# lez-s/Materialist

Hardware: AMD Instinct MI355X
Metric: opt_iterations_per_sec_512x512 (higher is better)
Workload: dtype f32; 1 GPU; BASELINE configs[1] synthetic: 1x512x512/GPU, --model_name pos_mlp --opt_order 'rm a' part rm, spp 64; mode=pos_mlp, height=512, width=512, spp=64, images_per_gpu=1, light=SH25, parallelism=dp1 (independent images, no data-path collective)

## Files before the change

### materialist_amd/csrc/posmlp_kernels.hip

```cpp
#include <hip/hip_runtime.h>
#include <stdint.h>
#include <atomic>
#include <type_traits>

#include "../../include/matpbr.h"
#include "../../include/matpbr_experimental.h"
#include "posmlp_device.hpp"

namespace {


constexpr int kBM = 128, kBN = 128, kBK = 32;
constexpr int kPersistent = 512;
constexpr int EPI_SINCOS = 0, EPI_MULC = 1, EPI_BIAS = 2;

struct HeadArgs {
  const float* w;
  int ldw;
  const float* bias;
  ArmHead h;
};

__global__ __launch_bounds__(256) void mlp_tail_copy_kernel(float* __restrict__ out, int ldo, const float* __restrict__ tail, int ldt, long M, int N) {
  const int w = 256 - N;
// ... 1455 lines not shown
#pragma unroll
      for (int q = 0; q < 4; ++q) *reinterpret_cast<float4*>(sx + lane * 16 + 4 * ((q + lane) & 3)) = *reinterpret_cast<const float4*>(xs + 4 * ((q + lane) & 3));
    }
    float4 cvb[2][4];
    auto cv_load = [&](int b, float4 (&dst)[4]) {
      const float* src = p.cmul + (size_t)(row0 + wm * 64 + (b >> 2) * 32 + t_row) * p.ldo + wn * 128 + (b & 3) * 32 + t_col;
#pragma unroll
      for (int ps = 0; ps < 4; ++ps) dst[ps] = *reinterpret_cast<const float4*>(src + (size_t)(8 * ps) * p.ldo);
    };
    if (EPI == EPI_MULC) cv_load(0, cvb[0]);
    float hacc[4][5];
#pragma unroll
    for (int b = 0; b < 8; ++b) {
      const int mi = b >> 2, ni = b & 3;
      const size_t o0 = (size_t)(row0 + wm * 64 + mi * 32 + t_row) * p.ldo + wn * 128 + ni * 32 + t_col;
      if (EPI == EPI_MULC && b + 1 < 8) cv_load(b + 1, cvb[(b + 1) & 1]);
      if (HEAD && ni == 0) {
#pragma unroll
        for (int ps = 0; ps < 4; ++ps)
#pragma unroll
          for (int j = 0; j < 5; ++j) hacc[ps][j] = 0.f;
      }
      float second[16];
#pragma unroll
      for (int r = 0; r < 16; ++r) {
        float v = acc[mi][ni][r];
        if (BLK) v *= a_unscale;
        if (EPI == EPI_SINCOS) {
          const float pre = F16 ? __builtin_fmaf(v, kF16WUnscale, bn[ni]) : v + bn[ni];
          if (PK) v = sin_packed(pre);
          else sincos_cw(pre, v, second[r]);
        }
        scr[((r & 3) + 8 * (r >> 2) + 4 * lh) * kLd + li] = v;
      }
      float4 vrow[4];
#pragma unroll
      for (int ps = 0; ps < 4; ++ps) {
        float4 v = *reinterpret_cast<const float4*>(scr + (t_row + 8 * ps) * kLd + t_col);
        if (EPI == EPI_MULC) {
          float4 c4 = cvb[b & 1][ps];
          if (p.cmul_sin) c4 = cos_from_packed_sin(c4);
          v.x *= c4.x; v.y *= c4.y; v.z *= c4.z; v.w *= c4.w;
          csum4[ni].x += v.x; csum4[ni].y += v.y; csum4[ni].z += v.z; csum4[ni].w += v.w;
          if (BLK && !W0) omax = __builtin_fmaxf(__builtin_fmaxf(omax, __builtin_fmaxf(__builtin_fabsf(v.x), __builtin_fabsf(v.y))),
                                                   __builtin_fmaxf(__builtin_fabsf(v.z), __builtin_fabsf(v.w)));
        }
        if (EPI == EPI_SINCOS && !HEAD && ni == 3 && p.tail != nullptr && wn == 1) {
            const int col = 224 + t_col;
            const float* tl = p.tail + (size_t)(row0 + wm * 64 + mi * 32 + t_row + 8 * ps) * p.ldt - p.N;
            if (col >= p.N) v.x = tl[col];
            if (col + 1 >= p.N) v.y = tl[col + 1];
            if (col + 2 >= p.N) v.z = tl[col + 2];
            if (col + 3 >= p.N) v.w = tl[col + 3];
        }
        if (W0) *reinterpret_cast<float4*>(scr + (t_row + 8 * ps) * kLd + t_col) = v;
        else *reinterpret_cast<float4*>(p.out0 + o0 + (size_t)(8 * ps) * p.ldo) = v;
        vrow[ps] = v;
      }
      if (W0) {
#pragma unroll
        for (int ct = 0; ct < 2; ++ct)
#pragma unroll
          for (int kk = 0; kk < 8; ++kk)
            acc0[ni][ct] = __builtin_amdgcn_mfma_f32_16x16x4f32(scr[(4 * kk + (lane >> 4)) * kLd + 16 * ct + (lane & 15)],
                                                                sx[(mi * 32 + 4 * kk + (lane >> 4)) * 16 + (lane & 15)], acc0[ni][ct], 0, 0, 0);
      }
      if (HEAD) {
#pragma unroll
        for (int j = 0; j < 5; ++j) {
          const float4 w4 = *reinterpret_cast<const float4*>(sW4 + j * 256 + wn * 128 + ni * 32 + t_col);
#pragma unroll
          for (int ps = 0; ps < 4; ++ps)
            hacc[ps][j] = __builtin_fmaf(vrow[ps].x, w4.x, __builtin_fmaf(vrow[ps].y, w4.y, __builtin_fmaf(vrow[ps].z, w4.z, __builtin_fmaf(vrow[ps].w, w4.w, hacc[ps][j]))));
        }
      }
      if (EPI == EPI_SINCOS && !PK) {
#pragma unroll
        for (int r = 0; r < 16; ++r) scr[((r & 3) + 8 * (r >> 2) + 4 * lh) * kLd + li] = second[r];
#pragma unroll
        for (int ps = 0; ps < 4; ++ps)
          *reinterpret_cast<float4*>(p.out1 + o0 + (size_t)(8 * ps) * p.ldo) = *reinterpret_cast<const float4*>(scr + (t_row + 8 * ps) * kLd + t_col);
      }
      if (HEAD && ni == 3) {
#pragma unroll
        for (int ps = 0; ps < 4; ++ps)
#pragma unroll
          for (int j = 0; j < 5; ++j) {
            float v = hacc[ps][j];
            v = dpp_add_f<0x111>(v);
            v = dpp_add_f<0x112>(v);
            v = dpp_add_f<0x114>(v);
            if ((lane & 7) == 7) sComb[((wm * 64 + mi * 32 + t_row + 8 * ps) * 2 + wn) * 8 + j] = v;
          }
      }
    }
    if (HEAD) {
      __syncthreads();
      if (tid < kBM) {
        float v5[5];
#pragma unroll
        for (int j = 0; j < 5; ++j) v5[j] = (sComb[(tid * 2) * 8 + j] + sComb[(tid * 2 + 1) * 8 + j]) + hd.bias[j];
        arm_head_store(hd.h, (long)row0 + tid, v5);
      }
      __syncthreads();
    }
    if (BLK && !W0 && p.o_tmax != nullptr) {
      const float wmx = wave_max_lane63(omax);
      if (lane == 63) atomicMax(p.o_tmax + tile, __float_as_uint(wmx));
    }
    asm volatile("s_waitcnt lgkmcnt(0)" ::: "memory");
  }
  asm volatile("s_waitcnt vmcnt(0)" ::: "memory");
  if (W0) {
    const size_t slab = (size_t)blockIdx.x * 2 + wm;
#pragma unroll
    for (int ni = 0; ni < 4; ++ni)
#pragma unroll
      for (int ct = 0; ct < 2; ++ct)
#pragma unroll
        for (int r = 0; r < 4; ++r)
          p.w0_part[(slab * 16 + (lane & 15)) * 256 + wn * 128 + ni * 32 + 16 * ct + 4 * (lane >> 4) + r] = acc0[ni][ct][r];
  }
  if (EPI == EPI_MULC && p.colsum != nullptr) {
    float* sRed = reinterpret_cast<float*>(gx_smem);
    const int t_row = lane >> 3, t_col = (lane & 7) * 4;
    __syncthreads();
#pragma unroll
    for (int ni = 0; ni < 4; ++ni)
      *reinterpret_cast<float4*>(sRed + (wm * 8 + t_row) * 256 + wn * 128 + ni * 32 + t_col) = csum4[ni];
    __syncthreads();
    float t = 0.f;
#pragma unroll
    for (int sl = 0; sl < 16; ++sl) t += sRed[sl * 256 + tid];
    p.colsum[(size_t)blockIdx.x * 256 + tid] = t;
  }
}

constexpr int kWgStage = 2 * 3 * 2 * 256;
constexpr size_t kWgSmem = 2 * kWgStage * sizeof(uint4);
#ifndef MATPBR_WG_DEPTH
#define MATPBR_WG_DEPTH 2
#endif
constexpr int kWgDepth = MATPBR_WG_DEPTH;
constexpr int kWgThreads = 512;
__device__ __forceinline__ int wg_perm(int i) { return (i & 16) + 2 * (i & 7) + ((i >> 3) & 1); }
template <int NPROD, bool EARLY>
__device__ __forceinline__ void wgrad_bx_body(const float* __restrict__ G, int ldg, const float* __restrict__ X, int ldx,
                                              float* __restrict__ partial, long M, long rows_per_slab, uint4* sW, const unsigned* __restrict__ g_tmax) {
  constexpr bool F16 = NPROD == 3;
  constexpr int NP = F16 ? 2 : 3;
  const int tid = threadIdx.x, lane = tid & 63, wave = tid >> 6;
  const int nq = wave >> 1, kq = wave & 1, li = lane & 31, lh = lane >> 5;
  const long m_begin = (long)blockIdx.x * rows_per_slab;
  const long m_end = (m_begin + rows_per_slab < M) ? m_begin + rows_per_slab : M;
  const int steps = m_begin < m_end ? (int)((m_end - m_begin) / 16) : 0;
  float g_scale = 1.0f, g_unscale = 1.0f;
  if (F16 && steps > 0) {
    unsigned mb = 0;
    for (long t = m_begin / kBM; t <= (m_end - 1) / kBM; ++t) mb = g_tmax[t] > mb ? g_tmax[t] : mb;
    block_scale(mb, g_scale, g_unscale);
  }

  f32x16 acc[2][4];
#pragma unroll
  for (int ni = 0; ni < 2; ++ni)
#pragma unroll
    for (int ki = 0; ki < 4; ++ki)
#pragma unroll
      for (int r = 0; r < 16; ++r) acc[ni][ki][r] = 0.f;

  const int cp = tid & 255, sh = tid >> 8;
  const float* src = (cp >> 7) ? X + (m_begin + 8 * sh) * ldx + 2 * (cp & 127) : G + (m_begin + 8 * sh) * ldg + 2 * (cp & 127);
  const long ld = (cp >> 7) ? ldx : ldg;
  const float my_scale = (F16 && !(cp >> 7)) ? g_scale : 1.0f;
  uint4* sdst = sW + (((cp >> 7) * NP) * 2 + sh) * 256 + ((cp & 127) >> 3) * 16 + (cp & 7);
  float2 raw[kWgDepth][8];
  auto load_stage = [&](int slot, int step) {
#pragma unroll
    for (int j = 0; j < 8; ++j) raw[slot][j] = *reinterpret_cast<const float2*>(src + (16L * step + j) * ld);
  };
  auto split_store = [&](int slot, int buf) {
#pragma unroll
    for (int c = 0; c < 2; ++c) {
      uint4 pc[3];
      const float2* r = raw[slot];
#define MATPBR_COMP(v) (c == 0 ? (v).x : (v).y)
      if (F16) {
        split2h(MATPBR_COMP(r[0]) * my_scale, MATPBR_COMP(r[1]) * my_scale, pc[0].x, pc[1].x);
        split2h(MATPBR_COMP(r[2]) * my_scale, MATPBR_COMP(r[3]) * my_scale, pc[0].y, pc[1].y);
        split2h(MATPBR_COMP(r[4]) * my_scale, MATPBR_COMP(r[5]) * my_scale, pc[0].z, pc[1].z);
        split2h(MATPBR_COMP(r[6]) * my_scale, MATPBR_COMP(r[7]) * my_scale, pc[0].w, pc[1].w);
      } else {
        split3(MATPBR_COMP(r[0]), MATPBR_COMP(r[1]), pc[0].x, pc[1].x, pc[2].x);
        split3(MATPBR_COMP(r[2]), MATPBR_COMP(r[3]), pc[0].y, pc[1].y, pc[2].y);
        split3(MATPBR_COMP(r[4]), MATPBR_COMP(r[5]), pc[0].z, pc[1].z, pc[2].z);
        split3(MATPBR_COMP(r[6]), MATPBR_COMP(r[7]), pc[0].w, pc[1].w, pc[2].w);
      }
#undef MATPBR_COMP
#pragma unroll
      for (int piece = 0; piece < NP; ++piece) sdst[buf * kWgStage + (piece * 2) * 256 + 8 * c] = pc[piece];
    }
  };
  auto stage = [&](int slot, int buf, int next_stage) {
    __builtin_amdgcn_sched_barrier(0);
    split_store(slot, buf);
    __builtin_amdgcn_sched_barrier(0);
    load_stage(slot, next_stage < steps ? next_stage : steps - 1);
    __builtin_amdgcn_sched_barrier(0);
  };

  if (steps > 0) {
    load_stage(0, 0);
    split_store(0, 0);
#pragma unroll
    for (int d = 0; d < kWgDepth; ++d) {
      __builtin_amdgcn_sched_barrier(0);
      load_stage((1 + d) % kWgDepth, 1 + d < steps ? 1 + d : steps - 1);
    }
    __builtin_amdgcn_sched_barrier(0);
    __syncthreads();
    auto step = [&](auto u_tag, int st) {
        constexpr int u = decltype(u_tag)::value;
        const int cur = st & 1;
        if (EARLY) stage((u + 1) % kWgDepth, cur ^ 1, st + 1 + kWgDepth);
        const uint4* sa = sW + cur * kWgStage + lh * 256 + nq * 64 + li;
        const uint4* sb = sW + cur * kWgStage + (NP * 2 + lh) * 256 + kq * 128 + li;
        uint4 a[3][2];
#pragma unroll
        for (int piece = 0; piece < NP; ++piece)
#pragma unroll
          for (int ni = 0; ni < 2; ++ni) a[piece][ni] = sa[(piece * 2) * 256 + ni * 32];
#pragma unroll
        for (int kh = 0; kh < 2; ++kh) {
          uint4 b[3][2];
#pragma unroll
          for (int piece = 0; piece < NP; ++piece)
#pragma unroll
            for (int k2 = 0; k2 < 2; ++k2) b[piece][k2] = sb[(piece * 2) * 256 + (kh * 2 + k2) * 32];
          if constexpr (F16) {
#pragma unroll
            for (int t = 0; t < 3; ++t) {
              constexpr int ia[3] = {1, 0, 0}, ib[3] = {0, 1, 0};
#pragma unroll
              for (int k2 = 0; k2 < 2; ++k2)
#pragma unroll
                for (int ni = 0; ni < 2; ++ni)
                  acc[ni][kh * 2 + k2] = __builtin_amdgcn_mfma_f32_32x32x16_f16(__builtin_bit_cast(f16x8, a[ia[t]][ni]),
                                                                               __builtin_bit_cast(f16x8, b[ib[t]][k2]), acc[ni][kh * 2 + k2], 0, 0, 0);
            }
          }
#pragma unroll
          for (int t = 0; t < (F16 ? 0 : 9); ++t) {
            constexpr int ia[9] = {2, 1, 2, 2, 0, 1, 1, 0, 0}, ib[9] = {2, 2, 1, 0, 2, 1, 0, 1, 0};
            if (NPROD == 6 && t < 3) continue;
#pragma unroll
            for (int k2 = 0; k2 < 2; ++k2)
#pragma unroll
              for (int ni = 0; ni < 2; ++ni)
                acc[ni][kh * 2 + k2] = __builtin_amdgcn_mfma_f32_32x32x16_bf16(__builtin_bit_cast(bf16x8, a[ia[t]][ni]),
                                                                              __builtin_bit_cast(bf16x8, b[ib[t]][k2]), acc[ni][kh * 2 + k2], 0, 0, 0);
          }
        }
        if (!EARLY) stage((u + 1) % kWgDepth, cur ^ 1, st + 1 + kWgDepth);
        __syncthreads();
    };
    int st0 = 0;
    for (; st0 + kWgDepth <= steps; st0 += kWgDepth) {
      step(std::integral_constant<int, 0>{}, st0);
      if constexpr (kWgDepth > 1) step(std::integral_constant<int, 1>{}, st0 + 1);
      if constexpr (kWgDepth > 2) step(std::integral_constant<int, 2>{}, st0 + 2);
      if constexpr (kWgDepth > 3) step(std::integral_constant<int, 3>{}, st0 + 3);
    }
    if (st0 < steps) step(std::integral_constant<int, 0>{}, st0);
    if constexpr (kWgDepth > 2) if (st0 + 1 < steps) step(std::integral_constant<int, 1>{}, st0 + 1);
    if constexpr (kWgDepth > 3) if (st0 + 2 < steps) step(std::integral_constant<int, 2>{}, st0 + 2);
  }
  float* out = partial + (long)blockIdx.x * 256 * 256;
#pragma unroll
  for (int ni = 0; ni < 2; ++ni)
#pragma unroll
    for (int ki = 0; ki < 4; ++ki)
#pragma unroll
      for (int r = 0; r < 16; ++r) {
        const int n = nq * 64 + ni * 32 + wg_perm((r & 3) + 8 * (r >> 2) + 4 * lh);
        const int k = kq * 128 + ki * 32 + wg_perm(li);
        out[n * 256 + k] = F16 ? acc[ni][ki][r] * g_unscale : acc[ni][ki][r];
      }
}

template <int NPROD>
__global__ __launch_bounds__(kWgThreads, 1) void mlp_wgrad_bx(const float* __restrict__ G, int ldg, const float* __restrict__ X, int ldx,
                                                              float* __restrict__ partial, long M, long rows_per_slab, const unsigned* __restrict__ g_tmax) {
  extern __shared__ __align__(16) unsigned char wg_smem[];
  uint4* sW = reinterpret_cast<uint4*>(wg_smem);
  if (threadIdx.x >> 8)
    wgrad_bx_body<NPROD, true>(G, ldg, X, ldx, partial, M, rows_per_slab, sW, g_tmax);
  else
    wgrad_bx_body<NPROD, false>(G, ldg, X, ldx, partial, M, rows_per_slab, sW, g_tmax);
}

#ifndef MATPBR_WG_HX
#define MATPBR_WG_HX 1
#endif
constexpr int kHxRaw = 16 * 2 * 1024;
constexpr int kHxPieces = 2 * 2 * 2 * 256;
constexpr size_t kHxSmem = 3 * kHxRaw + kHxPieces * sizeof(uint4);
__global__ __launch_bounds__(kWgThreads, 1) void mlp_wgrad_hx(const float* __restrict__ G, int ldg, const float* __restrict__ X, int ldx,
                                                              float* __restrict__ partial, long M, long rows_per_slab, const unsigned* __restrict__ g_tmax) {
  extern __shared__ __align__(16) unsigned char hx_smem[];
  uint4* sP = reinterpret_cast<uint4*>(hx_smem + 3 * kHxRaw);
  const int tid = threadIdx.x, lane = tid & 63, wave = tid >> 6;
  const int nq = wave >> 1, kq = wave & 1, li = lane & 31, lh = lane >> 5;
  (void)rows_per_slab;
  const int tiles = (int)(M / kBM);
  const int t_first = tiles - 1 - (int)blockIdx.x;
  const int my_tiles = t_first >= 0 ? t_first / (int)gridDim.x + 1 : 0;
  const int steps = my_tiles * (kBM / 16);
  float g_scale = 1.0f, g_unscale = 1.0f;
  if (steps > 0) {
    unsigned mb = 0;
    for (int t = t_first; t >= 0; t -= (int)gridDim.x) mb = g_tmax[t] > mb ? g_tmax[t] : mb;
    block_scale(mb, g_scale, g_unscale);
  }
  f32x16 acc[2][4];
#pragma unroll
  for (int ni = 0; ni < 2; ++ni)
#pragma unroll
    for (int ki = 0; ki < 4; ++ki)
#pragma unroll
      for (int r = 0; r < 16; ++r) acc[ni][ki][r] = 0.f;
  if (steps > 0) {
    const int wave_u = __builtin_amdgcn_readfirstlane(wave);
    const bool loader = wave_u < 4;
    const unsigned lds0 = lds_byte_address(hx_smem);
    unsigned vg[4], vx[4];
#pragma unroll
    for (int j = 0; j < 4; ++j) {
      vg[j] = (unsigned)(j * ldg) * 4u + (unsigned)lane * 16u - 1024u * j;
      vx[j] = (unsigned)(j * ldx) * 4u + (unsigned)lane * 16u - 1024u * j;
    }
    auto issue = [&](int step, int buf) {
      const int sc = step < steps ? step : steps - 1;
      const long row = ((long)t_first - (long)(sc >> 3) * gridDim.x) * kBM + 16 * (7 - (sc & 7)) + 4 * wave_u;
      const unsigned dst = lds0 + (unsigned)buf * (unsigned)kHxRaw + (unsigned)wave_u * 4096u;
      glds16_x4v(G + row * ldg, vg[0], vg[1], vg[2], vg[3], dst);
      glds16_x4v(X + row * ldx, vx[0], vx[1], vx[2], vx[3], dst + 16u * 1024u);
    };
    const int cp = tid & 255, sh = tid >> 8;
    const float my_scale = (cp >> 7) ? 1.0f : g_scale;
    const unsigned raw_off = (unsigned)((cp >> 7) * 16 * 1024 + (8 * sh) * 1024 + (cp & 127) * 8);
    uint4* sdst = sP + (((cp >> 7) * 2) * 2 + sh) * 256 + ((cp & 127) >> 3) * 16 + (cp & 7);
    float2 raw[8];
    auto read_raw = [&](int buf) {
#pragma unroll
      for (int j = 0; j < 8; ++j) raw[j] = *reinterpret_cast<const float2*>(hx_smem + buf * kHxRaw + raw_off + j * 1024);
    };
    auto cut_store = [&]() {
#pragma unroll
      for (int c = 0; c < 2; ++c) {
        uint4 pc[2];
#define MATPBR_COMP(v) (c == 0 ? (v).x : (v).y)
        split2h(MATPBR_COMP(raw[0]) * my_scale, MATPBR_COMP(raw[1]) * my_scale, pc[0].x, pc[1].x);
        split2h(MATPBR_COMP(raw[2]) * my_scale, MATPBR_COMP(raw[3]) * my_scale, pc[0].y, pc[1].y);
        split2h(MATPBR_COMP(raw[4]) * my_scale, MATPBR_COMP(raw[5]) * my_scale, pc[0].z, pc[1].z);
        split2h(MATPBR_COMP(raw[6]) * my_scale, MATPBR_COMP(raw[7]) * my_scale, pc[0].w, pc[1].w);
#undef MATPBR_COMP
#pragma unroll
        for (int piece = 0; piece < 2; ++piece) sdst[(piece * 2) * 256 + 8 * c] = pc[piece];
      }
    };
    auto products = [&](const uint4 (&a)[2][2], const uint4 (&b)[2][4]) {
#pragma unroll
      for (int ki = 0; ki < 4; ++ki)
#pragma unroll
        for (int t = 0; t < 3; ++t) {
          constexpr int ia[3] = {1, 0, 0}, ib[3] = {0, 1, 0};
#pragma unroll
          for (int ni = 0; ni < 2; ++ni)
            acc[ni][ki] = __builtin_amdgcn_mfma_f32_32x32x16_f16(__builtin_bit_cast(f16x8, a[ia[t]][ni]), __builtin_bit_cast(f16x8, b[ib[t]][ki]), acc[ni][ki], 0, 0, 0);
        }
    };
    if (loader) { issue(0, 0); issue(1, 1); }
    if (loader) asm volatile("s_waitcnt vmcnt(8)" ::: "memory");
    asm volatile("s_barrier" ::: "memory");
    read_raw(0);
    cut_store();
    if (loader) issue(2, 2);
    const uint4* sa = sP + lh * 256 + nq * 64 + li;
    const uint4* sb = sP + (2 * 2 + lh) * 256 + kq * 128 + li;
    int nxt = 1;
    for (int st = 0; st < steps; ++st) {
      if (loader) asm volatile("s_waitcnt vmcnt(8)" ::: "memory");
      asm volatile("s_waitcnt lgkmcnt(0)\n\ts_barrier" ::: "memory");
      uint4 a[2][2], b[2][4];
#pragma unroll
      for (int piece = 0; piece < 2; ++piece) {
#pragma unroll
        for (int ni = 0; ni < 2; ++ni) a[piece][ni] = sa[(piece * 2) * 256 + ni * 32];
#pragma unroll
        for (int ki = 0; ki < 4; ++ki) b[piece][ki] = sb[(piece * 2) * 256 + ki * 32];
      }
      read_raw(nxt);
      asm volatile("s_waitcnt lgkmcnt(0)\n\ts_barrier" ::: "memory");
      if (loader) {
        issue(st + 3, nxt == 0 ? 2 : nxt - 1);
        __builtin_amdgcn_sched_barrier(0);
      }
      products(a, b);
      cut_store();
      nxt = nxt == 2 ? 0 : nxt + 1;
    }
    asm volatile("s_waitcnt vmcnt(0)" ::: "memory");
  }
  float* out = partial + (long)blockIdx.x * 256 * 256;
#pragma unroll
  for (int ni = 0; ni < 2; ++ni)
#pragma unroll
    for (int ki = 0; ki < 4; ++ki)
#pragma unroll
      for (int r = 0; r < 16; ++r) {
        const int n = nq * 64 + ni * 32 + wg_perm((r & 3) + 8 * (r >> 2) + 4 * lh);
        const int k = kq * 128 + ki * 32 + wg_perm(li);
        out[n * 256 + k] = acc[ni][ki][r] * g_unscale;
      }
}

constexpr size_t kBxSmem = 2 * kBxStage * sizeof(uint4) + 8 * 32 * kLd * sizeof(float);
constexpr size_t kBxSmemHead = kBxSmem + (5 * 256 + 128 * 2 * 8) * sizeof(float);
std::atomic<int> g_nt_gl{2};
std::atomic<int> g_nt_w0_gx{0};
inline bool gl_ok(const NtArgs& p) {
  return g_nt_gl.load(std::memory_order_relaxed) != 0 && p.K > 32 && (long)kBM * p.lda * 4 < (1l << 31);
}
template <auto Kernel>
bool lds_opt_in(size_t bytes) {
  static std::atomic<unsigned long long> done{0};
  int dev = 0;
  if (hipGetDevice(&dev) != hipSuccess) return false;
  const unsigned long long bit = 1ull << (dev & 63);
  if (done.load(std::memory_order_acquire) & bit) return true;
  if (hipFuncSetAttribute(reinterpret_cast<const void*>(Kernel), hipFuncAttributeMaxDynamicSharedMemorySize, (int)bytes) != hipSuccess) return false;
  done.fetch_or(bit, std::memory_order_release);
  return true;
}
template <int EPI, int NPROD, bool FULL>
bool launch_nt_bx_full(const NtArgs& p, const uint4* wsplit, unsigned grid, hipStream_t stream) {
  if constexpr (FULL) if (gl_ok(p)) {
    if (!lds_opt_in<&mlp_nt_bx<EPI, NPROD, true, false, false, true>>(kGlSmem)) return false;
    hipLaunchKernelGGL((mlp_nt_bx<EPI, NPROD, true, false, false, true>), dim3(grid), dim3(kBxThreads), kGlSmem, stream, p, wsplit, HeadArgs{});
    return true;
  }
  if (!lds_opt_in<&mlp_nt_bx<EPI, NPROD, FULL>>(kBxSmem)) return false;
  hipLaunchKernelGGL((mlp_nt_bx<EPI, NPROD, FULL>), dim3(grid), dim3(kBxThreads), kBxSmem, stream, p, wsplit, HeadArgs{});
  return true;
}
constexpr size_t kBxSmemW0 = kBxSmem + 8 * 32 * 16 * sizeof(float);
template <int NPROD>
bool launch_nt_bx_w0(const NtArgs& p, const uint4* wsplit, unsigned grid, hipStream_t stream) {
  if (gl_ok(p)) {
    constexpr size_t bytes = kGlSmem + 8 * 32 * 16 * sizeof(float);
    if (!lds_opt_in<&mlp_nt_bx<EPI_MULC, NPROD, true, false, true, true>>(bytes)) return false;
    hipLaunchKernelGGL((mlp_nt_bx<EPI_MULC, NPROD, true, false, true, true>), dim3(grid), dim3(kBxThreads), bytes, stream, p, wsplit, HeadArgs{});
    return true;
  }
  if (!lds_opt_in<&mlp_nt_bx<EPI_MULC, NPROD, true, false, true>>(kBxSmemW0)) return false;
  hipLaunchKernelGGL((mlp_nt_bx<EPI_MULC, NPROD, true, false, true>), dim3(grid), dim3(kBxThreads), kBxSmemW0, stream, p, wsplit, HeadArgs{});
  return true;
}
template <int NPROD>
bool launch_nt_bx_head(const NtArgs& p, const uint4* wsplit, const HeadArgs& hd, unsigned grid, hipStream_t stream) {
  if (gl_ok(p)) {
    constexpr size_t bytes = kGlSmem + (5 * 256 + 128 * 2 * 8) * sizeof(float);
    if (!lds_opt_in<&mlp_nt_bx<EPI_SINCOS, NPROD, true, true, false, true>>(bytes)) return false;
    hipLaunchKernelGGL((mlp_nt_bx<EPI_SINCOS, NPROD, true, true, false, true>), dim3(grid), dim3(kBxThreads), bytes, stream, p, wsplit, hd);
    return true;
  }
  if (!lds_opt_in<&mlp_nt_bx<EPI_SINCOS, NPROD, true, true>>(kBxSmemHead)) return false;
  hipLaunchKernelGGL((mlp_nt_bx<EPI_SINCOS, NPROD, true, true>), dim3(grid), dim3(kBxThreads), kBxSmemHead, stream, p, wsplit, hd);
  return true;
}
template <int EPI, int NPROD>
bool launch_nt_bx_one(const NtArgs& p, const uint4* wsplit, unsigned grid, hipStream_t stream) {
  if (p.N >= 256 || EPI == EPI_MULC || p.tail != nullptr) return launch_nt_bx_full<EPI, NPROD, true>(p, wsplit, grid, stream);
  return launch_nt_bx_full<EPI, NPROD, false>(p, wsplit, grid, stream);
}
template <int EPI, int NPROD, bool HEAD, bool PK>
bool launch_nt_gx_pk(const NtArgs& p, const uint4* wsplit, const HeadArgs& hd, unsigned grid, hipStream_t stream) {
  if (!lds_opt_in<&mlp_nt_gx<EPI, NPROD, HEAD, PK>>(kGxSmem)) return false;
  hipLaunchKernelGGL((mlp_nt_gx<EPI, NPROD, HEAD, PK>), dim3(grid), dim3(kGxThreads), kGxSmem, stream, p, wsplit, hd);
  return true;
}
template <int EPI, int NPROD, bool HEAD>
bool launch_nt_gx(const NtArgs& p, const uint4* wsplit, const HeadArgs& hd, unsigned grid, hipStream_t stream) {
  if constexpr (EPI == EPI_SINCOS) {
    if (p.out1 == nullptr) return launch_nt_gx_pk<EPI, NPROD, HEAD, true>(p, wsplit, hd, grid, stream);
  }
  return launch_nt_gx_pk<EPI, NPROD, HEAD, false>(p, wsplit, hd, grid, stream);
}
inline bool gx_ok(const NtArgs& p) { return g_nt_gl.load(std::memory_order_relaxed) == 2 && gl_ok(p); }
template <int EPI>
int launch_nt_bx(NtArgs p, const uint4* wsplit, int nprod, hipStream_t stream) {
  const int tiles = p.M / kBM;
  if (nprod == 3) {
    if constexpr (EPI != EPI_BIAS) {
      if (p.K > 32 && (long)kBM * p.lda * 4 < (1l << 31) && (p.N >= 256 || EPI == EPI_MULC || p.tail != nullptr) && (EPI != EPI_MULC || p.a_tmax != nullptr)) {
        const unsigned grid2 = (unsigned)(tiles < 512 ? tiles : 512);
        return launch_nt_gx<EPI, 3, false>(p, wsplit, HeadArgs{}, grid2, stream) ? (int)grid2 : -1;
      }
    }
    return -1;
  }
  if constexpr (EPI != EPI_BIAS) {
    if (gx_ok(p) && (p.N >= 256 || EPI == EPI_MULC || p.tail != nullptr)) {
      const unsigned grid2 = (unsigned)(tiles < 512 ? tiles : 512);
      const bool ok2 = nprod == 9 ? launch_nt_gx<EPI, 9, false>(p, wsplit, HeadArgs{}, grid2, stream) : launch_nt_gx<EPI, 6, false>(p, wsplit, HeadArgs{}, grid2, stream);
      return ok2 ? (int)grid2 : -1;
    }
  }
  const unsigned grid = (unsigned)(tiles < 256 ? tiles : 256);
  const bool ok = nprod == 9 ? launch_nt_bx_one<EPI, 9>(p, wsplit, grid, stream) : launch_nt_bx_one<EPI, 6>(p, wsplit, grid, stream);
  return ok ? (int)grid : -1;
}

inline unsigned nt_grid(long M, int N) {
  const long rt = (M + kBM - 1) / kBM;
  const long items = N > kBN ? ((rt + 7) / 8) * 16 : rt;
  return (unsigned)(items < kPersistent ? items : kPersistent);
}

inline bool aligned16(const void* p) { return (reinterpret_cast<uintptr_t>(p) & 15u) == 0; }

template <int EPI>
int launch_nt(NtArgs p, long M, hipStream_t stream) {
  const int halves = (p.N + kBN - 1) / kBN;
  const bool pipe = p.K > 224 && p.ldo >= halves * kBN && p.lda >= 256 && p.ldb >= 256 && M >= kBM;
  int groups = 0;
  long done = 0;
  if (pipe && halves == 2) {
    done = M / kBM * kBM;
    p.M = (int)done;
    const long rt = done / kBM;
    const unsigned grid = (unsigned)(rt < kPersistent ? rt : kPersistent);
    hipLaunchKernelGGL(mlp_gemm_nt_wide<EPI>, dim3(grid), dim3(256), 0, stream, p);
    groups += (int)grid;
  } else if (pipe) {
    done = M / kBM * kBM;
    p.M = (int)done;
    const unsigned grid = nt_grid(done, p.N);
    hipLaunchKernelGGL(mlp_gemm_nt_pipe<EPI>, dim3(grid), dim3(256), 0, stream, p);
    groups += (int)grid;
  }
  if (done < M) {
    NtArgs q = p;
    q.A = p.A + (size_t)done * p.lda;
    q.out0 = p.out0 + (size_t)done * p.ldo;
    if (p.out1) q.out1 = p.out1 + (size_t)done * p.ldo;
    if (p.cmul) q.cmul = p.cmul + (size_t)done * p.ldo;
    if (p.tail) q.tail = p.tail + (size_t)done * p.ldt;
    if (p.colsum) q.colsum = p.colsum + (size_t)groups * 256;
    q.M = (int)(M - done);
    const unsigned grid = nt_grid(M - done, p.N);
    hipLaunchKernelGGL(mlp_gemm_nt<EPI>, dim3(grid), dim3(256), 0, stream, q);
    groups += (int)grid;
  }
  return groups;
}

template <int EPI, int KP>
__global__ __launch_bounds__(256) void mlp_thin_k_kernel(const NtArgs p, int tiles) {
  __shared__ __align__(16) float scr_all[4][32 * kLd];
  __shared__ __align__(16) float sWt[256 * KP];
  const int lane = threadIdx.x & 63, wave = threadIdx.x >> 6, li = lane & 31, lh = lane >> 5;
  float* scr = scr_all[wave];
  constexpr int KS = KP / 2;
  for (int i = threadIdx.x; i < 256 * KP; i += 256) {
    const int nn = i / KP, k = i - nn * KP;
    sWt[i] = (nn < p.N && k < p.K) ? p.B[(size_t)nn * p.ldb + k] : 0.f;
  }
  float bn[8];
#pragma unroll
  for (int ni = 0; ni < 8; ++ni) bn[ni] = (EPI != EPI_MULC && ni * 32 + li < p.N) ? p.bias[ni * 32 + li] : 0.f;
  __syncthreads();
  const int t_row = lane >> 3, t_col = (lane & 7) * 4;
  float4 csum[8];
#pragma unroll
  for (int ni = 0; ni < 8; ++ni) csum[ni] = make_float4(0.f, 0.f, 0.f, 0.f);
  for (int tile = blockIdx.x * 4 + wave; tile < tiles; tile += gridDim.x * 4) {
    const int row0 = tile * 32;
    float av[KS];
    {
      const int m = row0 + li < p.M ? row0 + li : p.M - 1;
      const float4* ap = reinterpret_cast<const float4*>(p.A + (size_t)m * p.lda);
#pragma unroll
      for (int q = 0; q < KP / 4; ++q) {
        const float4 v = ap[q];
        av[2 * q] = lh ? v.y : v.x;
        av[2 * q + 1] = lh ? v.w : v.z;
      }
    }
    const bool full_rows = row0 + 32 <= p.M;
#pragma unroll
    for (int ni = 0; ni < 8; ++ni) {
      if (ni * 32 >= p.N) break;
      f32x16 acc;
#pragma unroll
      for (int r = 0; r < 16; ++r) acc[r] = 0.f;
      float wb[KS];
#pragma unroll
      for (int q = 0; q < KP / 4; ++q) {
        const float4 v = *reinterpret_cast<const float4*>(sWt + (ni * 32 + li) * KP + 4 * q);
        wb[2 * q] = lh ? v.y : v.x;
        wb[2 * q + 1] = lh ? v.w : v.z;
      }
#pragma unroll
      for (int sidx = 0; sidx < KS; ++sidx) acc = __builtin_amdgcn_mfma_f32_32x32x2f32(av[sidx], wb[sidx], acc, 0, 0, 0);
      float4 cv[4];
      const size_t o0 = (size_t)(row0 + t_row) * p.ldo + ni * 32 + t_col;
      if (EPI == EPI_MULC) {
#pragma unroll
        for (int ps = 0; ps < 4; ++ps)
          cv[ps] = (full_rows || row0 + t_row + 8 * ps < p.M) ? *reinterpret_cast<const float4*>(p.cmul + o0 + (size_t)(8 * ps) * p.ldo)
                                                            : make_float4(0.f, 0.f, 0.f, 0.f);
      }
      float second[16];
#pragma unroll
      for (int r = 0; r < 16; ++r) {
        float v = acc[r];
        if (EPI == EPI_SINCOS) {
          if (p.out1 == nullptr) v = sin_packed<true>(v + bn[ni]);
          else sincos_cw(v + bn[ni], v, second[r]);
        } else if (EPI == EPI_BIAS) v += bn[ni];
        scr[((r & 3) + 8 * (r >> 2) + 4 * lh) * kLd + li] = v;
      }
      const bool all_cols = ni * 32 + 32 <= p.N || p.tail != nullptr;
#pragma unroll
      for (int ps = 0; ps < 4; ++ps) {
        float4 v = *reinterpret_cast<const float4*>(scr + (t_row + 8 * ps) * kLd + t_col);
        const bool row_ok = full_rows || row0 + t_row + 8 * ps < p.M;
        if (EPI == EPI_MULC) {
          if (p.cmul_sin) cv[ps] = cos_from_packed_sin(cv[ps]);
          v.x *= cv[ps].x; v.y *= cv[ps].y; v.z *= cv[ps].z; v.w *= cv[ps].w;
          if (!row_ok) v = make_float4(0.f, 0.f, 0.f, 0.f);
          csum[ni].x += v.x; csum[ni].y += v.y; csum[ni].z += v.z; csum[ni].w += v.w;
        }
        if (row_ok)
          store4_upto(p.out0 + o0 + (size_t)(8 * ps) * p.ldo, v, p.N - (ni * 32 + t_col), all_cols);
      }
      if (EPI == EPI_SINCOS && p.out1 != nullptr) {
#pragma unroll
        for (int r = 0; r < 16; ++r) scr[((r & 3) + 8 * (r >> 2) + 4 * lh) * kLd + li] = second[r];
#pragma unroll
        for (int ps = 0; ps < 4; ++ps)
          if (full_rows || row0 + t_row + 8 * ps < p.M)
            store4_upto(p.out1 + o0 + (size_t)(8 * ps) * p.ldo, *reinterpret_cast<const float4*>(scr + (t_row + 8 * ps) * kLd + t_col),
                        p.N - (ni * 32 + t_col), all_cols);
      }
    }
  }
  if (EPI == EPI_MULC && p.colsum != nullptr) {
    __shared__ float red[32][256];
    __syncthreads();
#pragma unroll
    for (int ni = 0; ni < 8; ++ni) *reinterpret_cast<float4*>(&red[wave * 8 + t_row][ni * 32 + t_col]) = csum[ni];
    __syncthreads();
    float t = 0.f;
#pragma unroll
    for (int sl = 0; sl < 32; ++sl) t += red[sl][threadIdx.x];
    p.colsum[(size_t)blockIdx.x * 256 + threadIdx.x] = t;
  }
}
constexpr int kThinBlocks = 1024;
inline int thin_pad(int K) { return K <= 8 ? 8 : 16; }
template <int EPI>
int launch_thin_k(const NtArgs& p, hipStream_t stream) {
  const int tiles = (p.M + 31) / 32;
  const int grid = (tiles + 3) / 4 < kThinBlocks ? (tiles + 3) / 4 : kThinBlocks;
  if (p.K <= 8) hipLaunchKernelGGL((mlp_thin_k_kernel<EPI, 8>), dim3(grid), dim3(256), 0, stream, p, tiles);
  else hipLaunchKernelGGL((mlp_thin_k_kernel<EPI, 16>), dim3(grid), dim3(256), 0, stream, p, tiles);
  return grid;
}

template <int J, bool HEAD>
__global__ __launch_bounds__(256) void mlp_skinny_nt_kernel(const float* __restrict__ X, int ldx, const float* __restrict__ W, int ldw,
                                                            const float* __restrict__ bias, float* __restrict__ out, int ldo, long M, int K,
                                                            const ArmHead h) {
  const int lane = threadIdx.x & 63;
  const long wave = (long)blockIdx.x * 4 + (threadIdx.x >> 6), waves = (long)gridDim.x * 4;
  const int k0 = 4 * lane;
  const bool in = k0 < K;
  float4 w[J];
#pragma unroll
  for (int j = 0; j < J; ++j) w[j] = in ? *reinterpret_cast<const float4*>(W + (size_t)j * ldw + k0) : make_float4(0.f, 0.f, 0.f, 0.f);
  const long tiles = (M + 63) / 64;
  constexpr int R = 4;
  for (long tile = wave; tile < tiles; tile += waves) {
    const long row0 = tile * 64;
    float mine[J];
#pragma unroll
    for (int j = 0; j < J; ++j) mine[j] = 0.f;
    float4 x[R];
    auto load_rows = [&](int g) {
#pragma unroll
      for (int r = 0; r < R; ++r) {
        long m = row0 + g * R + r;
        m = m < M ? m : M - 1;
        x[r] = in ? *reinterpret_cast<const float4*>(X + m * ldx + k0) : make_float4(0.f, 0.f, 0.f, 0.f);
      }
    };
    load_rows(0);
    for (int g = 0; g < 64 / R; ++g) {
      float4 cur[R];
#pragma unroll
      for (int r = 0; r < R; ++r) cur[r] = x[r];
// ... 738 lines not shown
```

Measured before the change: 654.3 it/s.

## Interleave global-to-LDS loads and fp16 split with MFMAs in wgrad_hx loop

Restructures the mlp_wgrad_hx main loop so the eight per-step global-to-LDS loads and the scale/split/store of the next raw tile are spread across groups of three MFMAs. The goal is to overlap memory issue and VALU conversion with matrix math instead of running them as separate phases. It also moves the g_tmax reduction after the prologue loads, unrolled by eight, so its latency hides behind the first fetches. The raw read is moved after the second barrier, and the ring depth is parameterised. The cost is more complex scheduling and extra macro variants, and it depends on the compiler keeping the interleaving.

```diff
diff --git a/materialist_amd/csrc/posmlp_kernels.hip b/materialist_amd/csrc/posmlp_kernels.hip
--- a/materialist_amd/csrc/posmlp_kernels.hip
+++ b/materialist_amd/csrc/posmlp_kernels.hip
@@ -1781,26 +1781,61 @@
 #ifndef MATPBR_WG_HX
 #define MATPBR_WG_HX 1
 #endif
+#ifndef MATPBR_WG_SPREAD
+#define MATPBR_WG_SPREAD 1
+#endif
+#ifndef MATPBR_WG_LATE_RAW
+#define MATPBR_WG_LATE_RAW MATPBR_WG_SPREAD
+#endif
+#ifndef MATPBR_WG_ONE_BARRIER
+#define MATPBR_WG_ONE_BARRIER 0
+#endif
+#ifndef MATPBR_WG_RING
+#define MATPBR_WG_RING 3
+#endif
+constexpr int kHxRing = MATPBR_WG_RING;
+constexpr int kHxAhead = 8 * (kHxRing - 2);
 constexpr int kHxRaw = 16 * 2 * 1024;
 constexpr int kHxPieces = 2 * 2 * 2 * 256;
-constexpr size_t kHxSmem = 3 * kHxRaw + kHxPieces * sizeof(uint4);
+#if MATPBR_WG_SPREAD && MATPBR_WG_ONE_BARRIER
+constexpr int kHxPieceBufs = 2;
+#else
+constexpr int kHxPieceBufs = 1;
+#endif
+constexpr size_t kHxSmem = kHxRing * kHxRaw + kHxPieceBufs * kHxPieces * sizeof(uint4);
+static_assert(kHxSmem <= 160 * 1024, "mlp_wgrad_hx: more LDS than a CU has");
 __global__ __launch_bounds__(kWgThreads, 1) void mlp_wgrad_hx(const float* __restrict__ G, int ldg, const float* __restrict__ X, int ldx,
                                                               float* __restrict__ partial, long M, long rows_per_slab, const unsigned* __restrict__ g_tmax) {
   extern __shared__ __align__(16) unsigned char hx_smem[];
-  uint4* sP = reinterpret_cast<uint4*>(hx_smem + 3 * kHxRaw);
+  uint4* sP = reinterpret_cast<uint4*>(hx_smem + kHxRing * kHxRaw);
   const int tid = threadIdx.x, lane = tid & 63, wave = tid >> 6;
   const int nq = wave >> 1, kq = wave & 1, li = lane & 31, lh = lane >> 5;
   (void)rows_per_slab;
+  int grid_u = (int)gridDim.x;
+#if MATPBR_WG_SPREAD
+  asm volatile("" : "+s"(grid_u));
+#endif
   const int tiles = (int)(M / kBM);
   const int t_first = tiles - 1 - (int)blockIdx.x;
-  const int my_tiles = t_first >= 0 ? t_first / (int)gridDim.x + 1 : 0;
+  const int my_tiles = t_first >= 0 ? t_first / grid_u + 1 : 0;
   const int steps = my_tiles * (kBM / 16);
   float g_scale = 1.0f, g_unscale = 1.0f;
-  if (steps > 0) {
+  auto slab_scale = [&]() {
     unsigned mb = 0;
+#if MATPBR_WG_SPREAD
+    for (int j = 0; j < my_tiles; j += 8) {
+      unsigned v[8];
+#pragma unroll
+      for (int u = 0; u < 8; ++u) v[u] = g_tmax[t_first - (j + u < my_tiles ? j + u : j) * grid_u];
+#pragma unroll
+      for (int u = 0; u < 8; ++u) mb = v[u] > mb ? v[u] : mb;
+    }
+#else
     for (int t = t_first; t >= 0; t -= (int)gridDim.x) mb = g_tmax[t] > mb ? g_tmax[t] : mb;
+#endif
     block_scale(mb, g_scale, g_unscale);
-  }
+  };
+  if (steps > 0 && !MATPBR_WG_SPREAD) slab_scale();
   f32x16 acc[2][4];
 #pragma unroll
   for (int ni = 0; ni < 2; ++ni)
@@ -1815,18 +1850,32 @@
     unsigned vg[4], vx[4];
 #pragma unroll
     for (int j = 0; j < 4; ++j) {
-      vg[j] = (unsigned)(j * ldg) * 4u + (unsigned)lane * 16u - 1024u * j;
-      vx[j] = (unsigned)(j * ldx) * 4u + (unsigned)lane * 16u - 1024u * j;
-    }
+      vg[j] = (unsigned)(j * ldg) * 4u + (unsigned)lane * 16u - (MATPBR_WG_SPREAD ? 0u : 1024u * j);
+      vx[j] = (unsigned)(j * ldx) * 4u + (unsigned)lane * 16u - (MATPBR_WG_SPREAD ? 0u : 1024u * j);
+    }
+    struct HxSrc { const float* g; const float* x; unsigned dst; };
+    auto step_src = [&](int step, int buf) {
+      const int sc = step < steps ? step : steps - 1;
+      const long row = ((long)t_first - (long)(sc >> 3) * grid_u) * kBM + 16 * (7 - (sc & 7)) + 4 * wave_u;
+      return HxSrc{G + row * ldg, X + row * ldx, lds0 + (unsigned)buf * (unsigned)kHxRaw + (unsigned)wave_u * 4096u};
+    };
+    auto piece = [&](const HxSrc& s, auto p_tag) {
+      constexpr int p = decltype(p_tag)::value;
+      if constexpr (p < 4) glds16(s.g, vg[p], s.dst + 1024u * p);
+      else glds16(s.x, vx[p - 4], s.dst + 16u * 1024u + 1024u * (p - 4));
+    };
     auto issue = [&](int step, int buf) {
-      const int sc = step < steps ? step : steps - 1;
-      const long row = ((long)t_first - (long)(sc >> 3) * gridDim.x) * kBM + 16 * (7 - (sc & 7)) + 4 * wave_u;
-      const unsigned dst = lds0 + (unsigned)buf * (unsigned)kHxRaw + (unsigned)wave_u * 4096u;
-      glds16_x4v(G + row * ldg, vg[0], vg[1], vg[2], vg[3], dst);
-      glds16_x4v(X + row * ldx, vx[0], vx[1], vx[2], vx[3], dst + 16u * 1024u);
+      const HxSrc s = step_src(step, buf);
+#if MATPBR_WG_SPREAD
+      piece(s, std::integral_constant<int, 0>{}); piece(s, std::integral_constant<int, 1>{}); piece(s, std::integral_constant<int, 2>{}); piece(s, std::integral_constant<int, 3>{});
+      piece(s, std::integral_constant<int, 4>{}); piece(s, std::integral_constant<int, 5>{}); piece(s, std::integral_constant<int, 6>{}); piece(s, std::integral_constant<int, 7>{});
+#else
+      glds16_x4v(s.g, vg[0], vg[1], vg[2], vg[3], s.dst);
+      glds16_x4v(s.x, vx[0], vx[1], vx[2], vx[3], s.dst + 16u * 1024u);
+#endif
     };
     const int cp = tid & 255, sh = tid >> 8;
-    const float my_scale = (cp >> 7) ? 1.0f : g_scale;
+    float my_scale = (cp >> 7) ? 1.0f : g_scale;
     const unsigned raw_off = (unsigned)((cp >> 7) * 16 * 1024 + (8 * sh) * 1024 + (cp & 127) * 8);
     uint4* sdst = sP + (((cp >> 7) * 2) * 2 + sh) * 256 + ((cp & 127) >> 3) * 16 + (cp & 7);
     float2 raw[8];
@@ -1848,7 +1897,7 @@
         for (int piece = 0; piece < 2; ++piece) sdst[(piece * 2) * 256 + 8 * c] = pc[piece];
       }
     };
-    auto products = [&](const uint4 (&a)[2][2], const uint4 (&b)[2][4]) {
+    [[maybe_unused]] auto products = [&](const uint4 (&a)[2][2], const uint4 (&b)[2][4]) {
 #pragma unroll
       for (int ki = 0; ki < 4; ++ki)
 #pragma unroll
@@ -1859,35 +1908,93 @@
             acc[ni][ki] = __builtin_amdgcn_mfma_f32_32x32x16_f16(__builtin_bit_cast(f16x8, a[ia[t]][ni]), __builtin_bit_cast(f16x8, b[ib[t]][ki]), acc[ni][ki], 0, 0, 0);
         }
     };
-    if (loader) { issue(0, 0); issue(1, 1); }
-    if (loader) asm volatile("s_waitcnt vmcnt(8)" ::: "memory");
+#if MATPBR_WG_SPREAD
+    auto scaled = [&](float v) { float r; asm("v_mul_f32 %0, %1, %2" : "=v"(r) : "v"(v), "v"(my_scale)); return r; };
+    int pw = 0;
+    uint4 pc[2];
+    auto cut_part = [&](auto q_tag) {
+      constexpr int q = decltype(q_tag)::value, c = q >> 1;
+#define MATPBR_COMP(v) (c == 0 ? (v).x : (v).y)
+      if constexpr ((q & 1) == 0) {
+        split2h(scaled(MATPBR_COMP(raw[0])), scaled(MATPBR_COMP(raw[1])), pc[0].x, pc[1].x);
+        split2h(scaled(MATPBR_COMP(raw[2])), scaled(MATPBR_COMP(raw[3])), pc[0].y, pc[1].y);
+      } else {
+        split2h(scaled(MATPBR_COMP(raw[4])), scaled(MATPBR_COMP(raw[5])), pc[0].z, pc[1].z);
+        split2h(scaled(MATPBR_COMP(raw[6])), scaled(MATPBR_COMP(raw[7])), pc[0].w, pc[1].w);
+#pragma unroll
+        for (int piece = 0; piece < 2; ++piece) sdst[pw + (piece * 2) * 256 + 8 * c] = pc[piece];
+      }
+#undef MATPBR_COMP
+    };
+    auto group = [&](const HxSrc& s, const uint4 (&a)[2][2], const uint4 (&b)[2][4], auto p_tag) {
+      constexpr int p = decltype(p_tag)::value;
+      constexpr int ia[3] = {1, 0, 0}, ib[3] = {0, 1, 0};
+      if (loader) piece(s, p_tag);
+#pragma unroll
+      for (int i = 3 * p; i < 3 * p + 3; ++i) {
+        const int t = i >> 3, ki = (i & 7) >> 1, ni = i & 1;
+        acc[ni][ki] = __builtin_amdgcn_mfma_f32_32x32x16_f16(__builtin_bit_cast(f16x8, a[ia[t]][ni]), __builtin_bit_cast(f16x8, b[ib[t]][ki]), acc[ni][ki], 0, 0, 0);
+      }
+      if constexpr (p >= 4) cut_part(std::integral_constant<int, p - 4>{});
+    };
+#endif
+    if (loader) {
+#pragma unroll
+      for (int r = 0; r < kHxRing - 1; ++r) issue(r, r);
+    }
+#if MATPBR_WG_SPREAD
+    slab_scale();
+    my_scale = (cp >> 7) ? 1.0f : g_scale;
+#endif
+    if (loader) asm volatile("s_waitcnt vmcnt(%0)" :: "n"(kHxAhead) : "memory");
     asm volatile("s_barrier" ::: "memory");
     read_raw(0);
     cut_store();
-    if (loader) issue(2, 2);
+    if (loader) issue(kHxRing - 1, kHxRing - 1);
     const uint4* sa = sP + lh * 256 + nq * 64 + li;
     const uint4* sb = sP + (2 * 2 + lh) * 256 + kq * 128 + li;
     int nxt = 1;
     for (int st = 0; st < steps; ++st) {
-      if (loader) asm volatile("s_waitcnt vmcnt(8)" ::: "memory");
+      if (loader) asm volatile("s_waitcnt vmcnt(%0)" :: "n"(kHxAhead) : "memory");
       asm volatile("s_waitcnt lgkmcnt(0)\n\ts_barrier" ::: "memory");
       uint4 a[2][2], b[2][4];
+#if MATPBR_WG_SPREAD && MATPBR_WG_ONE_BARRIER
+      const int pr = (st & 1) * kHxPieces;
+      pw = kHxPieces - pr;
+#else
+      constexpr int pr = 0;
+#endif
 #pragma unroll
       for (int piece = 0; piece < 2; ++piece) {
 #pragma unroll
-        for (int ni = 0; ni < 2; ++ni) a[piece][ni] = sa[(piece * 2) * 256 + ni * 32];
-#pragma unroll
-        for (int ki = 0; ki < 4; ++ki) b[piece][ki] = sb[(piece * 2) * 256 + ki * 32];
-      }
+        for (int ni = 0; ni < 2; ++ni) a[piece][ni] = sa[pr + (piece * 2) * 256 + ni * 32];
+#pragma unroll
+        for (int ki = 0; ki < 4; ++ki) b[piece][ki] = sb[pr + (piece * 2) * 256 + ki * 32];
+      }
+#if MATPBR_WG_SPREAD && MATPBR_WG_ONE_BARRIER
       read_raw(nxt);
+#else
+      if (!MATPBR_WG_LATE_RAW) read_raw(nxt);
       asm volatile("s_waitcnt lgkmcnt(0)\n\ts_barrier" ::: "memory");
+      if (MATPBR_WG_LATE_RAW) read_raw(nxt);
+#endif
+#if MATPBR_WG_SPREAD
+      {
+        const HxSrc s = step_src(st + kHxRing, nxt == 0 ? kHxRing - 1 : nxt - 1);
+        group(s, a, b, std::integral_constant<int, 0>{}); group(s, a, b, std::integral_constant<int, 1>{});
+        group(s, a, b, std::integral_constant<int, 2>{}); group(s, a, b, std::integral_constant<int, 3>{});
+        group(s, a, b, std::integral_constant<int, 4>{}); group(s, a, b, std::integral_constant<int, 5>{});
+        group(s, a, b, std::integral_constant<int, 6>{}); group(s, a, b, std::integral_constant<int, 7>{});
+      }
+#else
       if (loader) {
-        issue(st + 3, nxt == 0 ? 2 : nxt - 1);
+        issue(st + kHxRing, nxt == 0 ? kHxRing - 1 : nxt - 1);
         __builtin_amdgcn_sched_barrier(0);
       }
       products(a, b);
       cut_store();
-      nxt = nxt == 2 ? 0 : nxt + 1;
+#endif
+      nxt = nxt == kHxRing - 1 ? 0 : nxt + 1;
     }
     asm volatile("s_waitcnt vmcnt(0)" ::: "memory");
   }
```

New measurement: 657.4 it/s, median of 5. Within noise of the previous version (+0.5%).
